# btracey/mpi

Measured on AMD Instinct MI355X. Metric: allreduce_sum_f32_256MiB algbw, higher is better.
Workload: dtype f32; 1 GPU; BASELINE cfg 4: allreduce-sum f32 256 MiB/rank, 8 ranks; ranks=8, ranks_per_gpu=8, bytes_per_rank=268435456, algo=auto (library), schedule_by=library defaults (ranks meet on the host: one schedule), transport=intra-HBM (all ranks share one GPU)

## Files before the change

mpi_amd/build.py:

```python
from __future__ import annotations

import hashlib
import json
import os
import shutil
import subprocess
import sys

ROOT = os.path.dirname(os.path.dirname(os.path.abspath(__file__)))
CSRC = os.path.join(ROOT, "mpi_amd", "csrc")
LIB = os.path.join(ROOT, "mpi_amd", "libxmpi.so")
HOSTLIB = os.path.join(ROOT, "mpi_amd", "libxmpi_host.so")
BIN = os.path.join(ROOT, "mpi_amd", "bin")

HIPCC = os.environ.get("HIPCC") or shutil.which("hipcc") or "/opt/rocm/bin/hipcc"
ARCH = "gfx950"
CXXFLAGS = ["-O3", "-std=c++17", "-fPIC", "-ffp-contract=off", "-Wall", "-Wextra"]

LIB_SOURCES = ["kernels.hip", "sched.hip", "ll.hip", "engine.cpp", "p2p.cpp", "agent.cpp", "api.cpp", "pool.cpp", "init.cpp", "tune.cpp", "local.cpp", "dump.cpp", "ctl.cpp", "ctl_selftest.cpp", "plan.cpp", "zcopy.cpp", "heap.cpp", "dsync.cpp", "dsync_conn.cpp", "trace.cpp"]
LIB_HEADERS = ["kernels.h", "kdev.h", "sched_steps.h", "comm.h", "ctl.h", "plan.h", "trace.h", os.path.join("..", "..", "include", "xmpi.h"),
               os.path.join("..", "..", "include", "xmpi_test.h")]


MANIFEST = os.path.join(ROOT, "mpi_amd", ".build_manifest.json")
# ... 80 lines not shown
    if os.path.exists(mpi_cpp):
        deps = [mpi_cpp, net_cpp, os.path.join(host_dir, "mpi.hpp"), os.path.join(host_dir, "network.hpp"),
                os.path.join(host_dir, "gobwire.hpp"), os.path.join(ROOT, "include", "xmpi.h"),
                os.path.join(ROOT, "include", "xmpi_test.h")]
        if force or _newer(HOSTLIB, deps):
            _run(["g++", "-O2", "-std=c++17", "-fPIC", "-ffp-contract=off", "-fno-fast-math", "-Wall", "-Wextra", "-shared", *inc, mpi_cpp, net_cpp, "-o", HOSTLIB,
                  "-L", os.path.dirname(LIB), "-lxmpi", "-Wl,-rpath,$ORIGIN", "-lpthread"], HOSTLIB, deps)
        outs.append(HOSTLIB)
        for name, src in (("helloworld", os.path.join(ROOT, "examples", "helloworld.cpp")),
                          ("bounce", os.path.join(ROOT, "examples", "bounce.cpp")),
                          ("allreduce", os.path.join(ROOT, "examples", "allreduce.cpp")),
                          ("coll_sweep", os.path.join(ROOT, "examples", "coll_sweep.cpp")),
                          ("allreduce_bench", os.path.join(ROOT, "examples", "allreduce_bench.cpp")),
                          ("cfg5_sweep", os.path.join(ROOT, "examples", "cfg5_sweep.cpp")),
                          ("cfg3_allgather", os.path.join(ROOT, "examples", "cfg3_allgather.cpp")),
                          ("alltoall", os.path.join(ROOT, "examples", "alltoall.cpp"))):
            if os.path.exists(src):
                out = os.path.join(BIN, name)
                if force or _newer(out, [src] + deps):
                    _run(["g++", "-O2", "-std=c++17", "-Wall", "-Wextra", *inc, src, "-o", out, "-L",
                          os.path.dirname(LIB), "-lxmpi_host", "-lxmpi", "-Wl,-rpath,$ORIGIN/..", "-lpthread"],
                         out, [src] + deps)
                outs.append(out)
    launcher = os.path.join(ROOT, "launcher", "xmpirun.cpp")
    if os.path.exists(launcher):
        out = os.path.join(BIN, "xmpirun")
        if force or _newer(out, [launcher]):
            _run(["g++", "-O2", "-std=c++17", "-Wall", "-Wextra", launcher, "-o", out], out, [launcher])
        outs.append(out)
    return outs


def build_oracle(force: bool = False) -> list[str]:
    odir = os.path.join(ROOT, "oracle")
    outs = []
    src = os.path.join(odir, "xmpi_oracle.c")
    out = os.path.join(odir, "liboracle.so")
    if force or _newer(out, [src, os.path.join(odir, "xmpi_oracle.h")]):
        _run(["gcc", "-O2", "-std=c11", "-fPIC", "-shared", "-ffp-contract=off", "-fno-fast-math", "-Wall",
              "-Wextra", src, "-o", out, "-lm"], out, [src, os.path.join(odir, "xmpi_oracle.h")])
    outs.append(out)
    ref = os.path.join(odir, "refpath.cpp")
    if os.path.exists(ref):
        out = os.path.join(odir, "librefpath.so")
        if force or _newer(out, [ref, os.path.join(odir, "gob_codec.h")]):
            _run(["g++", "-O2", "-std=c++17", "-fPIC", "-shared", "-Wall", "-Wextra", ref, "-o", out, "-lpthread"],
# ... 56 lines not shown
```

mpi_amd/csrc/api.cpp:

```cpp
#include <algorithm>
#include <cstdio>
#include <cstdlib>
#include <cstring>
#include <mutex>
#include <string>

#include "comm.h"
#include "kernels.h"

namespace xmpi {

static thread_local std::string g_last_error;
thread_local uint64_t t_api_call = 0;

void set_last_error(const std::string& s) { g_last_error = s; }

int hip_fail(hipError_t e, const char* what, const char* file, int line) {
  const char* base = strrchr(file, '/');
  g_last_error = std::string(what) + " failed: " + hipGetErrorString(e) + " (" + (base ? base + 1 : file) + ":" +
                 std::to_string(line) + ")";
  (void)hipGetLastError();
  return XMPI_ERR_HIP;
}

// ... 66 lines not shown
  }
  c->wq_cv.notify_all();
  return r;
}

void drain_worker(xmpi_comm* c) {
  if (t_in_worker || !c->worker_started) return;
  std::unique_lock<std::mutex> l(c->wq_mu);
  c->wq_cv.wait(l, [c] { return c->wq_busy == 0; });
}

void stop_worker(xmpi_comm* c) {
  if (!c->worker_started) return;
  drain_worker(c);
  {
    std::lock_guard<std::mutex> l(c->wq_mu);
    c->wq_stop = true;
  }
  c->wq_cv.notify_all();
  c->worker.join();
  c->worker_started = false;
}

static int collective_on_host_meeting_ranks(xmpi_comm* c, int coll, int algo, int root, const void* sendbuf, void* recvbuf, size_t count, int dtype,
                                            int op) {
  const size_t es = xmpi_dtype_size((xmpi_dtype)dtype);
  const bool zc_algo = algo == XMPI_ALGO_ZCOPY || algo == XMPI_ALGO_ZPUSH || algo == XMPI_ALGO_LL;
  if (c->size > 1 && (zc_algo || (algo == XMPI_ALGO_AUTO && c->zero_copy))) {
    bool done = false;
    int zrc = zero_copy_collective(c, coll, root, sendbuf, recvbuf, count, dtype, op, algo == XMPI_ALGO_ZPUSH, &done);
    if (zrc != XMPI_OK || done) return zrc;
  }
  if (zc_algo) algo = XMPI_ALGO_AUTO;
  if (algo == XMPI_ALGO_RING_PUSH) algo = XMPI_ALGO_RING;
  if (algo == XMPI_ALGO_RHD_PUSH) algo = XMPI_ALGO_RHD;
  if (algo == XMPI_ALGO_TREE_PUSH) algo = XMPI_ALGO_TREE;
  PlanParams pp;
  pp.coll = coll;
  pp.algo = algo;
  pp.size = c->size;
  pp.rank = c->rank;
  pp.root = root;
  pp.count = count;
  pp.elem_size = es;
  pp.channels = c->channels > 0 ? (int)c->channels : ring_channel_count(c->size);
  pp.lanes = c->lanes;
  const size_t total = count * es;
  size_t chunk = total;
  if (coll == COLL_ALLREDUCE) chunk = total / (size_t)c->size / (size_t)std::max(1, pp.channels);
  pp.piece_bytes = choose_piece(c, chunk);
  pp.fuse = 1;
  pp.fifo_depth = c->fifo_depth;
  pp.oneshot_bytes = (size_t)std::max<long>(0, c->oneshot_bytes);
  Plan plan;
  int rc = build_plan(pp, &plan);
// ... 65 lines not shown
  RoctxRange range("xmpi:%s algo=%s bytes=%zu rank=%d/%d", coll_name(coll), algo_name(algo), count * es, c->rank, c->size);
  std::lock_guard<std::mutex> g(c->coll_mu);
  if (dsync_takes(c, coll, algo))
    return dsync_collective(c, coll, root, sendbuf, recvbuf, count, dtype, op, c->local_stream, true, algo);
  const bool send_host = !is_device_pointer(sendbuf), recv_host = !is_device_pointer(recvbuf);
  if (send_host || recv_host) {
    const size_t send_bytes = coll_send_bytes(coll, c->size, count * es), recv_bytes = coll_recv_bytes(coll, c->size, count * es);
    const bool in_place = sendbuf == recvbuf && coll != COLL_ALLGATHER;
    void* up_recv = recv_host ? heap_alloc(c->device, recv_bytes) : nullptr;
    void* up_send = send_host && !(in_place && recv_host) ? heap_alloc(c->device, send_bytes) : nullptr;
    if ((recv_host && !up_recv) || (send_host && !(in_place && recv_host) && !up_send)) {
      if (up_recv) (void)heap_free(up_recv);
      if (up_send) (void)heap_free(up_send);
      (void)hipGetLastError();
      return collective_on_host_meeting_ranks(c, coll, algo, root, sendbuf, recvbuf, count, dtype, op);
    }
    void* drecv = recv_host ? up_recv : recvbuf;
    const void* dsend = !send_host ? sendbuf : (in_place && recv_host) ? drecv : up_send;
    auto done = [&](int rc) {
      if (up_recv) (void)heap_free(up_recv);
      if (up_send) (void)heap_free(up_send);
      return rc;
    };
    hipStream_t s = c->local_stream;
    const void* src_up = coll == COLL_BCAST ? (c->rank == root && recv_host ? recvbuf : nullptr) : (send_host ? sendbuf : nullptr);
    void* dst_up = coll == COLL_BCAST ? drecv : const_cast<void*>(dsend);
    if (src_up) {
      if (hipMemcpyAsync(dst_up, src_up, send_bytes, hipMemcpyHostToDevice, s) != hipSuccess || hipStreamSynchronize(s) != hipSuccess)
        return done(hip_fail(hipGetLastError(), "hipMemcpyAsync(host slice -> its stand-in)", __FILE__, __LINE__));
    }
    int rc = collective_on_host_meeting_ranks(c, coll, algo, root, dsend, drecv, count, dtype, op);
    if (rc == XMPI_OK && recv_host && (coll != COLL_REDUCE || c->rank == root)) {
      if (hipMemcpyAsync(recvbuf, drecv, recv_bytes, hipMemcpyDeviceToHost, s) != hipSuccess || hipStreamSynchronize(s) != hipSuccess)
        rc = hip_fail(hipGetLastError(), "hipMemcpyAsync(stand-in -> host slice)", __FILE__, __LINE__);
    }
    return done(rc);
  }
  return collective_on_host_meeting_ranks(c, coll, algo, root, sendbuf, recvbuf, count, dtype, op);
}

}

using namespace xmpi;

static int why_peer(xmpi_comm* c, int rc, const char* what) {
  if (rc == XMPI_ERR_PEER && c->ctl) set_last_error(std::string(what) + ": " + c->ctl->abort_reason());
  return rc;
}

extern "C" {

size_t xmpi_dtype_size(xmpi_dtype dtype) {
  switch (dtype) {
    case XMPI_U8: return 1;
    case XMPI_I32: return 4;
    case XMPI_I64: return 8;
    case XMPI_F16: return 2;
// ... 485 lines not shown
    const int rc = collective(c, COLL_ALLREDUCE, algo, 0, sendbuf, recvbuf, count, (int)dtype, (int)op);
    if (rc != XMPI_OK) return rc;
  }
  return XMPI_OK;
}

int xmpi_heap_selftest(uint64_t seed, int rounds) { return heap_selftest(seed, rounds); }


int xmpi_set_param(xmpi_comm* c, const char* name, long value) {
  if (!c || c->finalized || !name) return XMPI_ERR_STATE;
  std::lock_guard<std::mutex> g(c->coll_mu);
  const std::string n = name;
  if (n == "channels") c->channels = std::max<long>(0, value);
  else if (n == "piece_bytes") c->piece_bytes = std::max<long>(0, value);
  else if (n == "copy_engine") c->copy_engine = value ? 1 : 0;
  else if (n == "timeout_s") c->timeout_s = value;
  else if (n == "prof_every") c->prof_every = std::max<long>(1, value);
  else if (n == "batch_copies") c->batch_copies = value ? 1 : 0;
  else if (n == "oneshot_bytes") c->oneshot_bytes = std::max<long>(0, value);
  else if (n == "zero_copy") c->zero_copy = value ? 1 : 0;
  else if (n == "zc_bcast_push_bytes") c->zc_bcast_push_bytes = std::max<long>(0, value);
  else if (n == "zc_group_launch") c->zc_group_launch = value ? 1 : 0;
  else if (n == "p2p_direct_bytes") c->p2p_direct_bytes = value;
  else if (n == "p2p_kernel_ack") c->p2p_kernel_ack = value ? 1 : 0;
  else if (n == "p2p_agent_us") c->p2p_agent_us = std::max<long>(0, value);
  else if (n == "dsync") c->dsync = value ? 1 : 0;
  else if (n == "dsync_grid") c->dsync_grid_cap = std::max<long>(0, value);
  else if (n == "dsync_unroll") c->dsync_unroll = std::max<long>(1, std::min<long>(2, value));
  else if (n == "dsync_tiles") c->dsync_tiles = std::max<long>(1, value);
  else if (n == "p2p_grid_cap") c->p2p_grid_cap = std::max<long>(0, std::min<long>(value, 4096));
  else if (n == "ll_bytes") c->ll_bytes = std::max<long>(0, std::min<long>((long)kLLMaxPayload, value));
  else if (n == "agent_ll") c->agent_ll = value < 0 ? 0 : std::min<long>(value, 2);
  else if (n == "ll_agent_us") c->ll_agent_us = std::max<long>(0, value);
  else if (n == "agent_ll_bytes") c->agent_ll_bytes = std::max<long>(0, std::min<long>((long)kLLMaxPayload, value));
  else if (n == "dsync_split_bytes") c->dsync_split_bytes = std::max<long>(0, value);
  else if (n == "xcd_check") c->xcd_check = value ? 1 : 0;
  else if (n == "body_sys") c->body_sys = value ? 1 : 0;
  else if (n == "xcds") c->xcds = (int)std::max<long>(0, std::min<long>(value, 32));
  else if (n == "sched_channels") c->sched_channels = std::max<long>(0, value);
  else if (n == "sched_grid") c->sched_grid = std::max<long>(0, value);
  else if (n == "tree_piece_bytes") c->tree_piece_bytes = std::max<long>(4096, value);
  else if (n == "tuned") c->tuned = value != 0;
  else if (n == "tune_mask") c->tune_mask = value;
  else if (n.rfind("tune_", 0) == 0) {
    int coll = -1, cls = -1;
// ... 95 lines not shown
  if (n == "tune_check_us") return (long)(c->tune_check_ms * 1e3);
  if (n.rfind("tune_", 0) == 0) {
    int coll = -1, cls = -1;
    char what[16] = {0};
    if (sscanf(name, "tune_%15[a-z]_%d_%d", what, &coll, &cls) == 3 && coll >= 0 && coll < 4 && cls >= 0 && cls < xmpi_comm::kTuneClasses) {
      const std::string w = what;
      if (w == "algo") return c->tune_algo[coll][cls];
      if (w == "split") return c->tune_split[coll][cls];
      if (w == "unroll") return c->tune_unroll[coll][cls];
    }
    return -1;
  }
  if (n.rfind("prof_min_ns_", 0) == 0 || n.rfind("prof_max_ns_", 0) == 0) {
    const int kind = name[12] - '0';
    if (kind < 0 || kind >= PROF_KINDS || name[13]) return -1;
    return (long)((n[6] == 'i' ? c->prof[kind].min_ms : c->prof[kind].max_ms) * 1e6);
  }
  if (n == "p2p_direct_count") return (long)c->p2p_direct_count;
  if (n == "p2p_staged_count") return (long)c->p2p_staged_count;
  if (n == "p2p_lane_count") return (long)c->p2p_lane_count;
  if (n == "host_bounce_calls") return (long)c->host_bounce_calls;
  if (n == "host_lane_bytes") return (long)c->ctl->host_lane_bytes();
  if (n == "zc_seq") return (long)c->zc_seq;
  if (n == "zc_fallbacks_unregistered") return (long)c->zc_fallbacks_unregistered;
  if (n == "zc_fallbacks_unmappable") return (long)c->zc_fallbacks_unmappable;
  if (n == "shared_stream") return c->shared_stream ? 1 : 0;
  if (n == "kernel_mode") return get_kernel_mode();
  if (n == "last_run_us") return (long)c->last_run_us;
  if (n == "last_sync_us") return (long)c->last_sync_us;
  if (n == "lanes") return c->lanes;
  if (n == "fifo_depth") return c->fifo_depth;
  if (n == "slot_bytes") return (long)c->slot_bytes;
  if (n == "p2p_slot_bytes") return (long)c->p2p_slot_bytes;
  if (n == "window_bytes") return (long)c->window_bytes;
  if (n == "ring_channels_max") return ring_channel_count(c->size) * c->lanes;
  if (n == "ring_channels") return ring_channel_count(c->size);
  return -1;
}

}
```

mpi_amd/csrc/comm.h:

```cpp
#pragma once
#include <hip/hip_runtime_api.h>

#include <atomic>
#include <condition_variable>
#include <cstring>
#include <deque>
#include <functional>
#include <map>
#include <thread>
#include <mutex>
#include <set>
#include <string>
#include <utility>
#include <vector>

#include "../../include/xmpi.h"
#include "../../include/xmpi_test.h"
#include "ctl.h"
#include "kernels.h"
#include "trace.h"
#include "plan.h"

namespace xmpi {

// ... 45 lines not shown
  std::string degraded_why;

  int lanes = 2, fifo_depth = 8, p2p_depth = 2;
  size_t slot_bytes = 4u << 20, p2p_slot_bytes = 4u << 20;
  size_t coll_region_bytes = 0;
  size_t coll_slot_off(int src, int lane, uint64_t seq) const {
    return (((size_t)src * lanes + lane) * fifo_depth + (size_t)(seq % (uint64_t)fifo_depth)) * slot_bytes;
  }
  size_t p2p_slot_off(int src, int entry, uint64_t seq) const {
    return coll_region_bytes +
           (((size_t)src * xmpi::kMailEntries + entry) * p2p_depth + (size_t)(seq % (uint64_t)p2p_depth)) *
               p2p_slot_bytes;
  }

  hipStream_t send_stream[xmpi::kMaxRanks] = {nullptr};
  hipStream_t recv_stream[xmpi::kMaxRanks] = {nullptr};
  hipStream_t local_stream = nullptr;
  hipStream_t batch_send_stream = nullptr, batch_recv_stream = nullptr;
  long zero_copy = 1;
  long zc_bcast_push_bytes = 256 << 10;
  long zc_group_launch = 1;
  uint64_t zc_fallbacks_unregistered = 0, zc_fallbacks_unmappable = 0;
  uint64_t zc_seq = 0;
  std::set<std::pair<uint64_t, uint64_t>> zc_announced;
  std::mutex zc_mu;
  long p2p_direct_bytes = 1;
  uint64_t p2p_direct_count = 0, p2p_staged_count = 0, p2p_lane_count = 0;
  uint64_t zc_retired_seen[xmpi::kMaxRanks] = {0};
  long oneshot_bytes = 1 << 20;
  long batch_copies = 1;
  bool shared_stream = false;
  bool staged_streams = false;
  bool peer_coloc[xmpi::kMaxRanks] = {false};
  long prof_every = 1;
  uint64_t prof_seq[xmpi::PROF_KINDS] = {0};

  long dsync = 1;
  bool dsync_ok = false;
  xmpi::DsyncPage* dpage = nullptr;
  xmpi::DsyncPage* peer_page[xmpi::kMaxRanks] = {nullptr};
  bool peer_page_opened[xmpi::kMaxRanks] = {false};
  const int32_t* dsync_abort_dev = nullptr;
  char* ctl_dev = nullptr;
  bool ctl_registered = false;
  xmpi::DsyncResolved* dsync_res = nullptr;
  hipEvent_t dsync_order_ev = nullptr;
// ... 134 lines not shown

  std::mutex ev_mu;
  std::vector<hipEvent_t> ev_free, ev_timed_free;

  bool prof_on = false;
  xmpi::ProfCounter prof[xmpi::PROF_KINDS];

  std::mutex coll_mu;
  std::mutex p2p_mu;
  std::set<std::pair<int, int>> send_tags, recv_tags;
  std::map<std::pair<int, int>, xmpi::MailEntry*> pending_sends;
  std::vector<hipStream_t> p2p_streams;

  std::thread worker;
  std::mutex wq_mu;
  std::condition_variable wq_cv;
  std::deque<std::pair<std::function<int()>, xmpi_request*>> wq;
  size_t wq_busy = 0;
  bool wq_stop = false, worker_started = false;
  bool finalized = false;
};

namespace xmpi {
int ensure_streams(xmpi_comm* c);
int run_plan(xmpi_comm* c, const Plan& plan, const void* sendbuf, void* recvbuf, int dtype, int op);
int p2p_send(xmpi_comm* c, const void* buf, size_t bytes, int dtype, int dest, int tag, bool wait_ack = true);
int p2p_wait(xmpi_comm* c, int dest, int tag);
int p2p_recv(xmpi_comm* c, void* buf, size_t cap_bytes, int dtype, int src, int tag, size_t* got_bytes);
int p2p_probe(xmpi_comm* c, int src, int tag, size_t* bytes, int* dtype);
bool agent_submit(xmpi_comm* c, void* dst, const void* from, size_t bytes, MailEntry* m);
void p2p_agent_stop(xmpi_comm* c);
int agent_submit_ll(xmpi_comm* c, const void* send, void* recv, size_t bytes, int ll_coll, int root, int dtype, int op, bool consecutive);
extern thread_local uint64_t t_api_call;
void ll_agent_stop(xmpi_comm* c);
int zero_copy_collective(xmpi_comm* c, int coll, int root, const void* sendbuf, void* recvbuf, size_t count,
                         int dtype, int op, bool push, bool* done, int iters = 1);
int registry_add(void* base, size_t bytes, int device);
void registry_remove(xmpi_comm* c, void* base);
void zc_close_peers(const xmpi_comm* c);
bool zc_export(xmpi_comm* c, const void* p, size_t need, BufRef* ref);
bool zc_import(xmpi_comm* c, int peer, const BufRef& ref, void** out);
bool registry_alive(uint64_t gen);
hipError_t ipc_open_shared(int owner_pid, uint64_t owner_addr, const void* handle_bytes, void** out);
void ipc_close_shared(void* ptr);
void* pool_acquire(int device, size_t bytes, int kind, bool* fresh, uint64_t* mark);
void pool_release(void* ptr, uint64_t mark = 0);
hipError_t pool_handle(void* ptr, void* handle_out);
hipStream_t stream_acquire(int device);
void stream_release(int device, hipStream_t s);
hipStream_t shared_stream_for(int device);
bool trace_on();
#define XMPI_TRACE_STEP(rank, what)                                                                          \
  do {                                                                                                       \
    if (::xmpi::trace_on()) fprintf(stderr, "[xmpi %d %.6f] %s\n", (rank), ::xmpi::now_seconds(), (what)); \
  } while (0)
long env_long(const char* name, long dflt);
inline int use_device(const xmpi_comm* c) {
  XMPI_HIP(hipSetDevice(c->device));
  return XMPI_OK;
}
#define XMPI_ENTER(c)                          \
  do {                                         \
    if (!(c) || (c)->finalized) {              \
      ::xmpi::set_last_error("communicator not initialised"); \
      return XMPI_ERR_STATE;                   \
    }                                          \
    int _rc = ::xmpi::use_device(c);           \
    if (_rc) return _rc;                       \
    ::xmpi::t_api_call = (c)->api_calls.fetch_add(1, std::memory_order_relaxed) + 1; \
  } while (0)
inline double wait_limit(const xmpi_comm* c) { return c->timeout_s > 0 ? (double)c->timeout_s : 1e18; }
void drain_worker(xmpi_comm* c);
void stop_worker(xmpi_comm* c);
// ... 47 lines not shown
```

mpi_amd/csrc/ctl.h:

```cpp
#pragma once
#include <atomic>
#include <cstddef>
#include <cstdint>
#include <string>

namespace xmpi {

constexpr int kMaxRanks = 16;
constexpr int kMaxLanes = 4;
constexpr int kMailEntries = 4;
constexpr int kHostLaneSlots = 4;
constexpr uint64_t kCtlMagic = 0x584D504943544C31ull;
constexpr uint32_t kCtlVersion = 11;

struct alignas(64) Counter {
  std::atomic<uint64_t> v;
  char pad[56];
};

struct PipeCtl {
  Counter head;
  Counter tail;
};

enum MailState : uint32_t { MAIL_FREE = 0, MAIL_CLAIMED = 1, MAIL_POSTED = 2, MAIL_MATCHED = 3, MAIL_DONE = 4 };

struct BufRef {
  uint64_t base;
  uint64_t gen;
  uint64_t offset;
  uint64_t bytes;
  uint8_t handle[64];
};

enum MailDirect : int32_t {
  DIRECT_NONE = 0,
// ... 21 lines not shown
  int32_t device;
  int32_t maps;
  uint64_t window_addr;
  uint64_t window_bytes;
  uint8_t ipc_handle[64];
  char busid[32];
  uint64_t flag_addr;
  uint64_t flag_epoch;
  uint8_t flag_handle[64];
  char maps_why[96];
  int64_t ll_choice;
  uint64_t start_time;
};
constexpr int32_t kMapsWindows = 1, kMapsFlags = 2;

struct alignas(64) BufDesc {
  std::atomic<uint64_t> seq;
  int32_t ok;
  int32_t fresh;
  std::atomic<int32_t> verdict;
  int32_t in_place;
  BufRef send, recv;
  uint32_t sig;
};
static_assert(sizeof(BufDesc) == 256, "a descriptor is four cache lines");

constexpr int kRetireRing = 512;
struct alignas(64) RetireLog {
  std::atomic<uint64_t> count;
  uint64_t gen[kRetireRing];
};

constexpr int kPubRing = 64;
struct PubEntry {
  uint64_t gen;
  uint64_t base;
  uint64_t bytes;
  uint64_t reserved;
  uint8_t handle[64];
};
struct alignas(64) PubTable {
  std::atomic<uint64_t> count;
  char pad[56];
  PubEntry e[kPubRing];
};

// ... 101 lines not shown
```

mpi_amd/csrc/init.cpp:

```cpp
#include <unistd.h>

#include <algorithm>
#include <cstdlib>
#include <cstring>
#include <string>

#include "comm.h"
#include "kernels.h"

namespace xmpi {
namespace {

void* zeroed_device_words(size_t bytes, hipStream_t s) {
  void* p = nullptr;
  if (hipMalloc(&p, bytes) == hipSuccess) (void)hipMemsetAsync(p, 0, bytes, s);
  else p = nullptr;
  (void)hipGetLastError();
  return p;
}

void release_mappings_and_streams(xmpi_comm* c) {
  zc_close_peers(c);
  dsync_finalize(c);
  for (int p = 0; p < c->size; p++) {
// ... 42 lines not shown
    (void)hipGetLastError();
    set_last_error("xmpi_init: no HIP device is visible; xmpi has no CPU fallback");
    return XMPI_ERR_NOGPU;
  }
  if (*device < 0) *device = rank % ndev;
  if (*device >= ndev) {
    set_last_error("xmpi_init: device " + std::to_string(*device) + " does not exist (" + std::to_string(ndev) + " visible)");
    return XMPI_ERR_ARG;
  }
  XMPI_HIP(hipSetDevice(*device));
  return XMPI_OK;
}

void read_env(xmpi_comm* c) {
  c->timeout_s = std::max<long>(0, env_long("XMPI_TIMEOUT_S", 0));
  c->channels = env_long("XMPI_CHANNELS", 0);
  c->piece_bytes = env_long("XMPI_PIECE_BYTES", 0);
  c->copy_engine = env_long("XMPI_COPY_ENGINE", 0);
  c->batch_copies = env_long("XMPI_BATCH_COPIES", 1) ? 1 : 0;
  c->oneshot_bytes = std::max<long>(0, env_long("XMPI_ONESHOT_BYTES", 1 << 20));
  c->zero_copy = env_long("XMPI_ZERO_COPY", 1) ? 1 : 0;
  c->zc_bcast_push_bytes = std::max<long>(0, env_long("XMPI_ZC_BCAST_PUSH_BYTES", 256 << 10));
  c->zc_group_launch = env_long("XMPI_ZC_GROUP_LAUNCH", 1) ? 1 : 0;
  c->p2p_direct_bytes = env_long("XMPI_P2P_DIRECT_BYTES", 1);
  if (getenv("XMPI_KERNEL_MODE")) set_kernel_mode((int)env_long("XMPI_KERNEL_MODE", -1));
  if (getenv("XMPI_GRID_CAP")) set_grid_cap((int)env_long("XMPI_GRID_CAP", 0));
  c->dsync = env_long("XMPI_DSYNC", 1) ? 1 : 0;
  c->dsync_split_bytes = std::max<long>(0, env_long("XMPI_DSYNC_SPLIT_BYTES", 4 << 20));
  c->xcd_check = env_long("XMPI_XCD_CHECK", 1) ? 1 : 0;
  c->body_sys = env_long("XMPI_BODY_SYS", -1);
  c->ll_bytes = env_long("XMPI_LL_BYTES", -1);
  c->agent_ll = std::max<long>(0, std::min<long>(env_long("XMPI_AGENT_LL", 1), 2));
  c->agent_ll_bytes = std::max<long>(0, std::min<long>((long)kLLMaxPayload, env_long("XMPI_AGENT_LL_BYTES", 8192)));
  c->sched_channels = std::max<long>(0, env_long("XMPI_SCHED_CHANNELS", 0));
  c->sched_grid = std::max<long>(0, env_long("XMPI_SCHED_GRID", 0));
  c->tree_piece_bytes = std::max<long>(4096, env_long("XMPI_TREE_PIECE_BYTES", 256 << 10));
  c->dsync_grid_cap = std::max<long>(0, env_long("XMPI_DSYNC_GRID", 0));
  c->p2p_kernel_ack = env_long("XMPI_P2P_KERNEL_ACK", 1) ? 1 : 0;
  c->p2p_agent_us = std::max<long>(0, env_long("XMPI_P2P_AGENT_US", 40));
  c->ll_agent_us = std::max<long>(0, env_long("XMPI_LL_AGENT_US", c->p2p_agent_us));
  c->p2p_grid_cap = std::max<long>(0, std::min<long>(env_long("XMPI_P2P_GRID_CAP", 0), 4096));
  c->watchdog_ms = std::max<long>(0, env_long("XMPI_WATCHDOG_MS", 50));
  c->selfcheck = env_long("XMPI_SELFCHECK", -1);
}

int join_job(int rank, int size, int device, const char* job_key, double limit, xmpi_comm** out) {
// ... 276 lines not shown
```

mpi_amd/csrc/pool.cpp:

```cpp
#include <signal.h>

#include <cerrno>
#include <cstring>
#include <mutex>
#include <vector>

#include "comm.h"

namespace xmpi {

struct IpcMapping {
  int owner_pid;
  uint64_t owner_addr;
  uint8_t handle[64];
  void* ptr;
  int refs;
};
static std::mutex g_ipc_mu;
static std::vector<IpcMapping> g_ipc_map;

hipError_t ipc_open_shared(int owner_pid, uint64_t owner_addr, const void* handle_bytes, void** out) {
  std::lock_guard<std::mutex> g(g_ipc_mu);
  for (size_t i = 0; i < g_ipc_map.size(); i++) {
    IpcMapping& m = g_ipc_map[i];
// ... 155 lines not shown
int ensure_streams(xmpi_comm* c) {
  if (c->shared_stream || c->staged_streams) return XMPI_OK;
  bool ok = (c->batch_send_stream = stream_acquire(c->device)) && (c->batch_recv_stream = stream_acquire(c->device));
  for (int p = 0; p < c->size && ok; p++) {
    if (p == c->rank) continue;
    ok = (c->send_stream[p] = stream_acquire(c->device)) && (c->recv_stream[p] = stream_acquire(c->device));
  }
  if (!ok) return hip_fail(hipGetLastError(), "hipStreamCreate", __FILE__, __LINE__);
  c->staged_streams = true;
  return XMPI_OK;
}

hipStream_t shared_stream_for(int device) {
  static std::mutex mu;
  static std::vector<std::pair<int, hipStream_t>> streams;
  std::lock_guard<std::mutex> g(mu);
  for (auto& kv : streams)
    if (kv.first == device) return kv.second;
  hipStream_t s = nullptr;
  if (hipStreamCreateWithFlags(&s, hipStreamNonBlocking) != hipSuccess) return nullptr;
  streams.push_back({device, s});
  return s;
}
}
```

mpi_amd/csrc/zcopy.cpp:

```cpp
#include <dirent.h>
#include <signal.h>
#include <unistd.h>

#include <cerrno>

#include <algorithm>
#include <atomic>
#include <cstdio>
#include <cstring>
#include <map>
#include <mutex>
#include <vector>

#include "comm.h"
#include "kernels.h"

namespace xmpi {
namespace {

struct Alloc {
  uint64_t base;
  size_t bytes;
  int device;
  uint64_t gen;
  bool have_handle;
  hipIpcMemHandle_t handle;
};
std::mutex g_reg_mu;
std::map<uint64_t, Alloc> g_reg;
uint64_t g_next_gen = 1;

bool registry_lookup(const void* p, size_t need, int device, Alloc* out) {
  std::lock_guard<std::mutex> g(g_reg_mu);
  const uint64_t a = (uint64_t)(uintptr_t)p;
// ... 91 lines not shown
    XMPI_HIP(hipEventRecord(fin, c->local_stream));
    Backoff bo;
    for (;;) {
      const hipError_t e = hipEventQuery(fin);
      if (e == hipSuccess) break;
      if (e != hipErrorNotReady) return hip_fail(e, "hipEventQuery", __FILE__, __LINE__);
      (void)hipGetLastError();
      bo.pause();
    }
    ev_put(c, fin, false);
    if (start) {
      float ms = 0.f;
      XMPI_HIP(hipEventElapsedTime(&ms, start, stop));
      ProfCounter& pc = c->prof[PROF_ZCOPY];
      pc.add(ms, bytes);
      ev_put(c, start, true);
      ev_put(c, stop, true);
      start = stop = nullptr;
    }
    return XMPI_OK;
  }
};

}

int registry_add(void* base, size_t bytes, int device) {
  std::lock_guard<std::mutex> g(g_reg_mu);
  Alloc al;
  memset(&al, 0, sizeof al);
  al.base = (uint64_t)(uintptr_t)base;
  al.bytes = bytes;
  al.device = device;
  al.gen = g_next_gen++;
  al.have_handle = false;
  g_reg[al.base] = al;
  return XMPI_OK;
}

void registry_remove(xmpi_comm* c, void* base) {
  std::lock_guard<std::mutex> g(g_reg_mu);
  auto it = g_reg.find((uint64_t)(uintptr_t)base);
  if (it == g_reg.end()) return;
  if (it->second.have_handle && c && c->ctl) {
    RetireLog* log = c->ctl->retired(c->rank);
    const uint64_t n = log->count.load(std::memory_order_relaxed);
    log->gen[n % kRetireRing] = it->second.gen;
// ... 61 lines not shown
  }
  drop_retired(c);
  void* base = nullptr;
  if (map_peer(pid, ref, &base) != hipSuccess) return false;
  *out = (char*)base + ref.offset;
  return true;
}

void zc_close_peers(const xmpi_comm* c) {
  (void)c;
  std::lock_guard<std::mutex> g(g_map_mu);
  for (size_t i = 0; i < g_maps.size();) {
    if (kill(g_maps[i].pid, 0) != 0 && errno == ESRCH) {
      (void)hipIpcCloseMemHandle(g_maps[i].ptr);
      g_maps.erase(g_maps.begin() + (long)i);
    } else {
      i++;
    }
  }
  (void)hipGetLastError();
}

static int zc_run(xmpi_comm* c, int coll, int root, const void* sendbuf, void* recvbuf, size_t count, int dtype,
                  int op, bool push, bool* done, int iters) {
  *done = false;
  const int N = c->size, me = c->rank;
  const size_t es = xmpi_dtype_size((xmpi_dtype)dtype);
  const size_t unit = count * es;
  const size_t send_bytes = coll_send_bytes(coll, N, unit), recv_bytes = coll_recv_bytes(coll, N, unit);
  const bool recv_significant = (coll != COLL_REDUCE) || me == root;

  const uint64_t seq = ++c->zc_seq;
  BufDesc* mine = c->ctl->desc(me, seq);
  bool fresh = false;
  bool ok = fill_ref(c, sendbuf, send_bytes, &mine->send, &fresh);
  if (recv_significant) ok = fill_ref(c, recvbuf, recv_bytes, &mine->recv, &fresh) && ok;
  else mine->recv = mine->send;
  mine->ok = ok ? 1 : 0;
  mine->fresh = fresh ? 1 : 0;
  mine->in_place = (sendbuf == recvbuf) ? 1 : 0;
  {
    const bool reduces = coll_reduces(coll), rooted = coll == COLL_BCAST || coll == COLL_REDUCE;
    uint64_t h = 0x9E3779B97F4A7C15ull;
    for (uint64_t v : {(uint64_t)coll + 1, (uint64_t)(push ? 2 : 1), (uint64_t)send_bytes, reduces ? (uint64_t)dtype + 1 : 0,
                       reduces ? (uint64_t)op + 1 : 0, rooted ? (uint64_t)root + 1 : 0, (uint64_t)iters}) {
      h = (h ^ v) * 0x100000001B3ull;
      h ^= h >> 29;
    }
    mine->sig = (uint32_t)(h ^ (h >> 32));
  }
  mine->verdict.store(0, std::memory_order_relaxed);
  mine->seq.store(seq, std::memory_order_release);
  int rc = c->ctl->barrier(wait_limit(c));
  if (rc != XMPI_OK) {
    set_last_error("zero-copy collective: a peer did not arrive");
    return rc;
  }

  drop_retired(c);

  bool all_ok = true, any_fresh = false, any_in_place = false;
  for (int p = 0; p < N; p++) {
    BufDesc* d = c->ctl->desc(p, seq);
    if (d->seq.load(std::memory_order_acquire) != seq) {
      set_last_error("zero-copy collective: ranks disagree on the collective sequence (mismatched calls?)");
      c->ctl->set_abort(XMPI_ERR_STATE);
      return XMPI_ERR_STATE;
    }
    if (d->sig != mine->sig) {
      set_last_error("collective: the ranks are not in the same call (collective, length, dtype, operation or root differ between "
                     "this rank and a peer); nothing was moved");
      c->ctl->set_abort(XMPI_ERR_ARG);
      return XMPI_ERR_ARG;
    }
    all_ok = all_ok && d->ok == 1;
    any_fresh = any_fresh || d->fresh == 1;
    any_in_place = any_in_place || d->in_place == 1;
  }
  if (!all_ok) {
    c->zc_fallbacks_unregistered++;
    return XMPI_OK;
  }

  const int mypid = (int)getpid();
  char* psend[kMaxRanks];
  char* precv[kMaxRanks];
  bool mapped = true;
  for (int p = 0; p < N && mapped; p++) {
    if (p == me) {
      psend[p] = (char*)const_cast<void*>(sendbuf);
      precv[p] = (char*)recvbuf;
      continue;
    }
    const BufDesc* d = c->ctl->desc(p, seq);
    const int pid = c->ctl->info(p)->pid;
    if (pid == mypid) {
      psend[p] = (char*)(uintptr_t)(d->send.base + d->send.offset);
      precv[p] = (char*)(uintptr_t)(d->recv.base + d->recv.offset);
      continue;
    }
// ... 10 lines not shown
        fprintf(stderr, "xmpi: rank %d cannot map a buffer of rank %d (pid %d): %s; %zu mappings open, %d fds open\n",
                me, p, pid, hipGetErrorString(me_err), g_maps.size(), count_open_fds());
    }
    if (mapped) {
      psend[p] = (char*)bs + d->send.offset;
      precv[p] = (char*)br + d->recv.offset;
    }
  }
  if (any_fresh) {
    mine->verdict.store(mapped ? 1 : -1, std::memory_order_release);
    rc = c->ctl->barrier(wait_limit(c));
    if (rc != XMPI_OK) return rc;
    for (int p = 0; p < N; p++)
      if (c->ctl->desc(p, seq)->verdict.load(std::memory_order_acquire) != 1) {
        c->zc_fallbacks_unmappable++;
        return XMPI_OK;
      }
  } else if (!mapped) {
    set_last_error("zero-copy collective: a peer buffer that was mapped before can no longer be mapped");
    c->ctl->set_abort(XMPI_ERR_HIP);
    return XMPI_ERR_HIP;
  }

  hipStream_t s = c->local_stream;
  Launcher L(c);
  const size_t al = std::max<size_t>(1, 16 / es);
  const bool use_push = push && coll == COLL_ALLREDUCE && !any_in_place && N > 1 && count % ((size_t)N * al) == 0;
  if (use_push) {
    const size_t C = count / (size_t)N, cb = C * es;
    {
      void* dst[kMaxBatch];
      const void* src[kMaxBatch];
      size_t bytes[kMaxBatch];
      int n = 0;
      for (int d = 1; d < N; d++) {
        const int q = (me + d) % N;
        dst[n] = precv[q] + (size_t)me * cb;
        src[n] = psend[me] + (size_t)q * cb;
        bytes[n] = cb;
        if (++n == kMaxBatch || d == N - 1) {
          rc = L.begin(2 * (size_t)n * cb);
          if (rc) return rc;
          XMPI_HIP(launch_copy_batch(dst, nullptr, src, bytes, n, s, L.start, L.stop));
          rc = L.finish();
          if (rc) return rc;
          n = 0;
// ... 5 lines not shown
    {
      const void* srcs[kMaxRanks];
      for (int p = 0; p < N; p++) srcs[p] = (p == me) ? psend[me] + (size_t)me * cb : precv[me] + (size_t)p * cb;
      void* d1[1] = {precv[me] + (size_t)me * cb};
      rc = L.begin((size_t)(N + 1) * cb);
      if (rc) return rc;
      XMPI_HIP(launch_reduce_n_multi(d1, 1, srcs, N, C, dtype, op, s, L.start, L.stop));
      rc = L.finish();
      if (rc) return rc;
    }
    rc = c->ctl->barrier(wait_limit(c));
    if (rc != XMPI_OK) return rc;
    {
      void* dsts[kMaxRanks];
      int nd = 0;
      for (int d = 1; d < N; d++) dsts[nd++] = precv[(me + d) % N] + (size_t)me * cb;
      rc = L.begin((size_t)(1 + nd) * cb);
      if (rc) return rc;
      XMPI_HIP(launch_copy_multi(dsts, nd, precv[me] + (size_t)me * cb, cb, s, L.start, L.stop));
      rc = L.finish();
      if (rc) return rc;
    }
  } else if (coll == COLL_ALLREDUCE || coll == COLL_REDUCE) {
    int lo = me, hi = me;
    if (c->zc_group_launch) {
      while (lo > 0 && c->peer_coloc[lo - 1]) lo--;
      while (hi + 1 < N && c->peer_coloc[hi + 1]) hi++;
    }
    size_t off = 0, cnt = 0, off_hi = 0, cnt_hi = 0;
    zc_chunk(count, es, N, lo, &off, &cnt);
    zc_chunk(count, es, N, hi, &off_hi, &cnt_hi);
    cnt = off_hi + cnt_hi - off;
    if (me == lo && cnt > 0) {
      const void* srcs[kMaxRanks];
      void* dsts[kMaxRanks];
      for (int p = 0; p < N; p++) srcs[p] = psend[p] + off * es;
      int nd = 0;
      if (coll == COLL_REDUCE) {
        dsts[nd++] = precv[root] + off * es;
      } else {
        dsts[nd++] = precv[me] + off * es;
        for (int d = 1; d < N; d++) dsts[nd++] = precv[(me + d) % N] + off * es;
      }
      std::vector<std::pair<hipEvent_t, hipEvent_t>> sampled;
      for (int it = 0; it < iters; it++) {
        rc = L.begin((size_t)(N + nd) * cnt * es);
        if (rc) return rc;
        XMPI_HIP(launch_reduce_n_multi(dsts, nd, srcs, N, cnt, dtype, op, s, L.start, L.stop));
        if (it + 1 < iters && L.start) {
          sampled.push_back({L.start, L.stop});
          L.start = L.stop = nullptr;
        }
      }
      rc = L.finish();
      if (rc) return rc;
      for (auto& ev : sampled) {
        float ms = 0.f;
        XMPI_HIP(hipEventElapsedTime(&ms, ev.first, ev.second));
        ProfCounter& pc = c->prof[PROF_ZCOPY];
        pc.add(ms, (size_t)(N + nd) * cnt * es);
        ev_put(c, ev.first, true);
        ev_put(c, ev.second, true);
      }
    }
  } else if (coll == COLL_REDUCE_SCATTER) {
    const void* srcs[kMaxRanks];
    for (int p = 0; p < N; p++) srcs[p] = psend[p] + (size_t)me * unit;
    void* d1[1] = {precv[me]};
    rc = L.begin((size_t)(N + 1) * unit);
    if (rc) return rc;
    XMPI_HIP(launch_reduce_n_multi(d1, 1, srcs, N, count, dtype, op, s, L.start, L.stop));
    rc = L.finish();
    if (rc) return rc;
  } else if (coll == COLL_ALLTOALL) {
    static_assert(kMaxRanks <= kMaxBatch, "one batch holds a pair per rank");
    void* dst[kMaxBatch];
    const void* src[kMaxBatch];
    size_t bytes[kMaxBatch];
    for (int d = 0; d < N; d++) {
      const int q = (me + d) % N;
      dst[d] = precv[q] + (size_t)me * unit;
      src[d] = psend[me] + (size_t)q * unit;
      bytes[d] = unit;
    }
    rc = L.begin(2 * (size_t)N * unit);
    if (rc) return rc;
    XMPI_HIP(launch_copy_batch(dst, nullptr, src, bytes, N, s, L.start, L.stop));
// ... 62 lines not shown
          if (q != root) dsts[nd++] = precv[q] + off * es;
        }
        if (cnt > 0 && nd > 0) {
          rc = L.begin((size_t)(1 + nd) * cnt * es);
          if (rc) return rc;
          XMPI_HIP(launch_copy_multi(dsts, nd, precv[me] + off * es, cnt * es, s, L.start, L.stop));
          rc = L.finish();
          if (rc) return rc;
        }
      }
    }
  }

  rc = c->ctl->barrier(wait_limit(c));
  if (rc != XMPI_OK) {
    set_last_error("zero-copy collective: a peer did not finish");
    return rc;
  }
  *done = true;
  return XMPI_OK;
}

int zero_copy_collective(xmpi_comm* c, int coll, int root, const void* sendbuf, void* recvbuf, size_t count,
                         int dtype, int op, bool push, bool* done, int iters) {
  RoctxRange range("xmpi:zcopy(host rendezvous) %s count=%zu x%d", coll_name(coll), count, iters);
  const int rc = zc_run(c, coll, root, sendbuf, recvbuf, count, dtype, op, push, done, iters);
  if (rc != XMPI_OK) c->ctl->set_abort(rc);
  return rc;
}

}
```

Before: 396.3 GB/s.

## Pipeline host-slice allreduce in pieces overlapping upload, reduce, and download

When allreduce buffers live in host memory, the zero-copy path now splits the work into fixed-size pieces (8 MiB by default). The host-to-device upload of the next piece is interleaved with the reduction of the current one, and a background thread copies finished pieces back to the host on a separate stream. This targets the serial upload, reduce and download sequence for host buffers. It adds two barriers per piece, a helper thread, and a descriptor field so all ranks agree on the piece size.

```diff
diff --git a/mpi_amd/build.py b/mpi_amd/build.py
--- a/mpi_amd/build.py
+++ b/mpi_amd/build.py
@@ -126,6 +126,12 @@
                           os.path.dirname(LIB), "-lxmpi_host", "-lxmpi", "-Wl,-rpath,$ORIGIN/..", "-lpthread"],
                          out, [src] + deps)
                 outs.append(out)
+    duplex = os.path.join(ROOT, "examples", "pcie_duplex.cpp")
+    if os.path.exists(duplex):
+        out = os.path.join(BIN, "pcie_duplex")
+        if force or _newer(out, [duplex]):
+            _run([HIPCC, f"--offload-arch={ARCH}", "-O2", "-std=c++17", "-Wall", "-Wextra", duplex, "-o", out, "-lpthread"], out, [duplex])
+        outs.append(out)
     launcher = os.path.join(ROOT, "launcher", "xmpirun.cpp")
     if os.path.exists(launcher):
         out = os.path.join(BIN, "xmpirun")
diff --git a/mpi_amd/csrc/api.cpp b/mpi_amd/csrc/api.cpp
--- a/mpi_amd/csrc/api.cpp
+++ b/mpi_amd/csrc/api.cpp
@@ -112,15 +112,40 @@
   c->worker_started = false;
 }
 
+int host_leg_up(xmpi_comm* c, HostLeg* leg, size_t upto) {
+  upto = std::min(upto, leg->bytes);
+  if (!leg->up_src || leg->up_done >= upto) return XMPI_OK;
+  hipStream_t up = nullptr, down = nullptr;
+  if (!host_leg_streams(c->device, &up, &down)) return hip_fail(hipGetLastError(), "hipStreamCreate(host leg)", __FILE__, __LINE__);
+  XMPI_HIP(hipMemcpyAsync(leg->up_dst + leg->up_done, leg->up_src + leg->up_done, upto - leg->up_done, hipMemcpyHostToDevice, up));
+  XMPI_HIP(hipStreamSynchronize(up));
+  leg->up_done = upto;
+  return XMPI_OK;
+}
+
+static int rc_up_rest(xmpi_comm* c, HostLeg* leg) {
+  const int rc = host_leg_up(c, leg, leg->bytes);
+  if (rc != XMPI_OK) c->ctl->set_abort(rc);
+  return rc;
+}
+
+static size_t host_piece_for(const xmpi_comm* c, int coll, int algo, size_t count, size_t es) {
+  if (coll != COLL_ALLREDUCE || c->host_piece_bytes <= 0 || c->size < 2 || t_in_worker) return 0;
+  if (!(algo == XMPI_ALGO_ZCOPY || algo == XMPI_ALGO_LL || (algo == XMPI_ALGO_AUTO && c->zero_copy))) return 0;
+  const size_t piece = std::max<size_t>(4096, (size_t)c->host_piece_bytes / 4096 * 4096);
+  return count * es > piece ? piece : 0;
+}
+
 static int collective_on_host_meeting_ranks(xmpi_comm* c, int coll, int algo, int root, const void* sendbuf, void* recvbuf, size_t count, int dtype,
-                                            int op) {
+                                            int op, HostLeg* leg = nullptr) {
   const size_t es = xmpi_dtype_size((xmpi_dtype)dtype);
   const bool zc_algo = algo == XMPI_ALGO_ZCOPY || algo == XMPI_ALGO_ZPUSH || algo == XMPI_ALGO_LL;
   if (c->size > 1 && (zc_algo || (algo == XMPI_ALGO_AUTO && c->zero_copy))) {
     bool done = false;
-    int zrc = zero_copy_collective(c, coll, root, sendbuf, recvbuf, count, dtype, op, algo == XMPI_ALGO_ZPUSH, &done);
+    int zrc = zero_copy_collective(c, coll, root, sendbuf, recvbuf, count, dtype, op, algo == XMPI_ALGO_ZPUSH, &done, 1, leg);
     if (zrc != XMPI_OK || done) return zrc;
   }
+  if (leg && (rc_up_rest(c, leg)) != XMPI_OK) return XMPI_ERR_HIP;
   if (zc_algo) algo = XMPI_ALGO_AUTO;
   if (algo == XMPI_ALGO_RING_PUSH) algo = XMPI_ALGO_RING;
   if (algo == XMPI_ALGO_RHD_PUSH) algo = XMPI_ALGO_RHD;
@@ -232,17 +257,34 @@
       if (up_send) (void)heap_free(up_send);
       return rc;
     };
+    auto failed = [&](const char* what) {
+      const int rc = hip_fail(hipGetLastError(), what, __FILE__, __LINE__);
+      c->ctl->set_abort(rc);
+      return done(rc);
+    };
     hipStream_t s = c->local_stream;
     const void* src_up = coll == COLL_BCAST ? (c->rank == root && recv_host ? recvbuf : nullptr) : (send_host ? sendbuf : nullptr);
     void* dst_up = coll == COLL_BCAST ? drecv : const_cast<void*>(dsend);
-    if (src_up) {
+    HostLeg leg;
+    leg.piece = host_piece_for(c, coll, algo, count, es);
+    if (leg.piece) {
+      leg.bytes = count * es;
+      leg.up_src = (const char*)src_up;
+      leg.up_dst = (char*)dst_up;
+      leg.down_dst = recv_host ? (char*)recvbuf : nullptr;
+      leg.down_src = (const char*)drecv;
+      if (host_leg_up(c, &leg, leg.piece) != XMPI_OK) {
+        c->ctl->set_abort(XMPI_ERR_HIP);
+        return done(XMPI_ERR_HIP);
+      }
+    } else if (src_up) {
       if (hipMemcpyAsync(dst_up, src_up, send_bytes, hipMemcpyHostToDevice, s) != hipSuccess || hipStreamSynchronize(s) != hipSuccess)
-        return done(hip_fail(hipGetLastError(), "hipMemcpyAsync(host slice -> its stand-in)", __FILE__, __LINE__));
-    }
-    int rc = collective_on_host_meeting_ranks(c, coll, algo, root, dsend, drecv, count, dtype, op);
-    if (rc == XMPI_OK && recv_host && (coll != COLL_REDUCE || c->rank == root)) {
+        return failed("hipMemcpyAsync(host slice -> its stand-in)");
+    }
+    int rc = collective_on_host_meeting_ranks(c, coll, algo, root, dsend, drecv, count, dtype, op, leg.piece ? &leg : nullptr);
+    if (rc == XMPI_OK && recv_host && !leg.down_done && (coll != COLL_REDUCE || c->rank == root)) {
       if (hipMemcpyAsync(recvbuf, drecv, recv_bytes, hipMemcpyDeviceToHost, s) != hipSuccess || hipStreamSynchronize(s) != hipSuccess)
-        rc = hip_fail(hipGetLastError(), "hipMemcpyAsync(stand-in -> host slice)", __FILE__, __LINE__);
+        return failed("hipMemcpyAsync(stand-in -> host slice)");
     }
     return done(rc);
   }
@@ -774,6 +816,7 @@
   else if (n == "zero_copy") c->zero_copy = value ? 1 : 0;
   else if (n == "zc_bcast_push_bytes") c->zc_bcast_push_bytes = std::max<long>(0, value);
   else if (n == "zc_group_launch") c->zc_group_launch = value ? 1 : 0;
+  else if (n == "host_piece_bytes") c->host_piece_bytes = std::max<long>(0, value);
   else if (n == "p2p_direct_bytes") c->p2p_direct_bytes = value;
   else if (n == "p2p_kernel_ack") c->p2p_kernel_ack = value ? 1 : 0;
   else if (n == "p2p_agent_us") c->p2p_agent_us = std::max<long>(0, value);
@@ -915,6 +958,8 @@
   if (n == "host_bounce_calls") return (long)c->host_bounce_calls;
   if (n == "host_lane_bytes") return (long)c->ctl->host_lane_bytes();
   if (n == "zc_seq") return (long)c->zc_seq;
+  if (n == "host_piece_bytes") return c->host_piece_bytes;
+  if (n == "host_pieces") return (long)c->host_pieces;
   if (n == "zc_fallbacks_unregistered") return (long)c->zc_fallbacks_unregistered;
   if (n == "zc_fallbacks_unmappable") return (long)c->zc_fallbacks_unmappable;
   if (n == "shared_stream") return c->shared_stream ? 1 : 0;
diff --git a/mpi_amd/csrc/comm.h b/mpi_amd/csrc/comm.h
--- a/mpi_amd/csrc/comm.h
+++ b/mpi_amd/csrc/comm.h
@@ -91,6 +91,8 @@
   long zc_group_launch = 1;
   uint64_t zc_fallbacks_unregistered = 0, zc_fallbacks_unmappable = 0;
   uint64_t zc_seq = 0;
+  long host_piece_bytes = 8 << 20;
+  uint64_t host_pieces = 0;
   std::set<std::pair<uint64_t, uint64_t>> zc_announced;
   std::mutex zc_mu;
   long p2p_direct_bytes = 1;
@@ -271,6 +273,17 @@
 };
 
 namespace xmpi {
+struct HostLeg {
+  const char* up_src = nullptr;
+  char* up_dst = nullptr;
+  char* down_dst = nullptr;
+  const char* down_src = nullptr;
+  size_t bytes = 0;
+  size_t piece = 0;
+  size_t up_done = 0;
+  bool down_done = false;
+};
+int host_leg_up(xmpi_comm* c, HostLeg* leg, size_t upto);
 int ensure_streams(xmpi_comm* c);
 int run_plan(xmpi_comm* c, const Plan& plan, const void* sendbuf, void* recvbuf, int dtype, int op);
 int p2p_send(xmpi_comm* c, const void* buf, size_t bytes, int dtype, int dest, int tag, bool wait_ack = true);
@@ -283,7 +296,7 @@
 extern thread_local uint64_t t_api_call;
 void ll_agent_stop(xmpi_comm* c);
 int zero_copy_collective(xmpi_comm* c, int coll, int root, const void* sendbuf, void* recvbuf, size_t count,
-                         int dtype, int op, bool push, bool* done, int iters = 1);
+                         int dtype, int op, bool push, bool* done, int iters = 1, HostLeg* leg = nullptr);
 int registry_add(void* base, size_t bytes, int device);
 void registry_remove(xmpi_comm* c, void* base);
 void zc_close_peers(const xmpi_comm* c);
@@ -298,6 +311,7 @@
 hipStream_t stream_acquire(int device);
 void stream_release(int device, hipStream_t s);
 hipStream_t shared_stream_for(int device);
+bool host_leg_streams(int device, hipStream_t* up, hipStream_t* down);
 bool trace_on();
 #define XMPI_TRACE_STEP(rank, what)                                                                          \
   do {                                                                                                       \
diff --git a/mpi_amd/csrc/ctl.h b/mpi_amd/csrc/ctl.h
--- a/mpi_amd/csrc/ctl.h
+++ b/mpi_amd/csrc/ctl.h
@@ -11,7 +11,7 @@
 constexpr int kMailEntries = 4;
 constexpr int kHostLaneSlots = 4;
 constexpr uint64_t kCtlMagic = 0x584D504943544C31ull;
-constexpr uint32_t kCtlVersion = 11;
+constexpr uint32_t kCtlVersion = 12;
 
 struct alignas(64) Counter {
   std::atomic<uint64_t> v;
@@ -79,6 +79,7 @@
   int32_t in_place;
   BufRef send, recv;
   uint32_t sig;
+  uint64_t host_piece;
 };
 static_assert(sizeof(BufDesc) == 256, "a descriptor is four cache lines");
 
diff --git a/mpi_amd/csrc/init.cpp b/mpi_amd/csrc/init.cpp
--- a/mpi_amd/csrc/init.cpp
+++ b/mpi_amd/csrc/init.cpp
@@ -88,6 +88,7 @@
   c->zero_copy = env_long("XMPI_ZERO_COPY", 1) ? 1 : 0;
   c->zc_bcast_push_bytes = std::max<long>(0, env_long("XMPI_ZC_BCAST_PUSH_BYTES", 256 << 10));
   c->zc_group_launch = env_long("XMPI_ZC_GROUP_LAUNCH", 1) ? 1 : 0;
+  c->host_piece_bytes = std::max<long>(0, env_long("XMPI_HOST_PIECE_BYTES", 8l << 20));
   c->p2p_direct_bytes = env_long("XMPI_P2P_DIRECT_BYTES", 1);
   if (getenv("XMPI_KERNEL_MODE")) set_kernel_mode((int)env_long("XMPI_KERNEL_MODE", -1));
   if (getenv("XMPI_GRID_CAP")) set_grid_cap((int)env_long("XMPI_GRID_CAP", 0));
diff --git a/mpi_amd/csrc/pool.cpp b/mpi_amd/csrc/pool.cpp
--- a/mpi_amd/csrc/pool.cpp
+++ b/mpi_amd/csrc/pool.cpp
@@ -201,4 +201,30 @@
   streams.push_back({device, s});
   return s;
 }
-}
+
+bool host_leg_streams(int device, hipStream_t* up, hipStream_t* down) {
+  struct Pair {
+    int device;
+    hipStream_t up, down;
+  };
+  static std::mutex mu;
+  static std::vector<Pair> pairs;
+  std::lock_guard<std::mutex> g(mu);
+  for (auto& p : pairs)
+    if (p.device == device) {
+      *up = p.up;
+      *down = p.down;
+      return true;
+    }
+  Pair p{device, nullptr, nullptr};
+  if (hipStreamCreateWithFlags(&p.up, hipStreamNonBlocking) != hipSuccess) return false;
+  if (hipStreamCreateWithFlags(&p.down, hipStreamNonBlocking) != hipSuccess) {
+    (void)hipStreamDestroy(p.up);
+    return false;
+  }
+  pairs.push_back(p);
+  *up = p.up;
+  *down = p.down;
+  return true;
+}
+}
diff --git a/mpi_amd/csrc/zcopy.cpp b/mpi_amd/csrc/zcopy.cpp
--- a/mpi_amd/csrc/zcopy.cpp
+++ b/mpi_amd/csrc/zcopy.cpp
@@ -6,10 +6,12 @@
 
 #include <algorithm>
 #include <atomic>
+#include <condition_variable>
 #include <cstdio>
 #include <cstring>
 #include <map>
 #include <mutex>
+#include <thread>
 #include <vector>
 
 #include "comm.h"
@@ -147,6 +149,132 @@
   }
 };
 
+
+int zc_fold(xmpi_comm* c, Launcher& L, int coll, int root, char* const* psend, char* const* precv, size_t first, size_t n, size_t es,
+            int dtype, int op, int iters) {
+  const int N = c->size, me = c->rank;
+  hipStream_t s = c->local_stream;
+  int rc = XMPI_OK;
+  int lo = me, hi = me;
+  if (c->zc_group_launch) {
+    while (lo > 0 && c->peer_coloc[lo - 1]) lo--;
+    while (hi + 1 < N && c->peer_coloc[hi + 1]) hi++;
+  }
+  size_t off = 0, cnt = 0, off_hi = 0, cnt_hi = 0;
+  zc_chunk(n, es, N, lo, &off, &cnt);
+  zc_chunk(n, es, N, hi, &off_hi, &cnt_hi);
+  cnt = off_hi + cnt_hi - off;
+  off += first;
+  if (me == lo && cnt > 0) {
+    const void* srcs[kMaxRanks];
+    void* dsts[kMaxRanks];
+    for (int p = 0; p < N; p++) srcs[p] = psend[p] + off * es;
+    int nd = 0;
+    if (coll == COLL_REDUCE) {
+      dsts[nd++] = precv[root] + off * es;
+    } else {
+      dsts[nd++] = precv[me] + off * es;
+      for (int d = 1; d < N; d++) dsts[nd++] = precv[(me + d) % N] + off * es;
+    }
+    std::vector<std::pair<hipEvent_t, hipEvent_t>> sampled;
+    for (int it = 0; it < iters; it++) {
+      rc = L.begin((size_t)(N + nd) * cnt * es);
+      if (rc) return rc;
+      XMPI_HIP(launch_reduce_n_multi(dsts, nd, srcs, N, cnt, dtype, op, s, L.start, L.stop));
+      if (it + 1 < iters && L.start) {
+        sampled.push_back({L.start, L.stop});
+        L.start = L.stop = nullptr;
+      }
+    }
+    rc = L.finish();
+    if (rc) return rc;
+    for (auto& ev : sampled) {
+      float ms = 0.f;
+      XMPI_HIP(hipEventElapsedTime(&ms, ev.first, ev.second));
+      ProfCounter& pc = c->prof[PROF_ZCOPY];
+      pc.add(ms, (size_t)(N + nd) * cnt * es);
+      ev_put(c, ev.first, true);
+      ev_put(c, ev.second, true);
+    }
+  }
+  return XMPI_OK;
+}
+
+struct Downloader {
+  xmpi_comm* c;
+  HostLeg* leg;
+  hipStream_t stream;
+  size_t piece;
+  std::mutex mu;
+  std::condition_variable cv;
+  size_t released = 0;
+  bool stop = false;
+  int rc = XMPI_OK;
+  hipError_t err = hipSuccess;
+  std::thread th;
+  void main() {
+    if (hipSetDevice(c->device) != hipSuccess) return fail(hipGetLastError());
+    for (size_t p = 0; p * piece < leg->bytes; p++) {
+      {
+        std::unique_lock<std::mutex> l(mu);
+        cv.wait(l, [&] { return stop || released > p; });
+        if (released <= p) return;
+      }
+      const size_t off = p * piece, len = std::min(piece, leg->bytes - off);
+      if (hipMemcpyAsync(leg->down_dst + off, leg->down_src + off, len, hipMemcpyDeviceToHost, stream) != hipSuccess ||
+          hipStreamSynchronize(stream) != hipSuccess)
+        return fail(hipGetLastError());
+    }
+  }
+  void fail(hipError_t e) {
+    err = e;
+    rc = XMPI_ERR_HIP;
+    c->ctl->set_abort(rc);
+  }
+  void release(size_t n) {
+    {
+      std::lock_guard<std::mutex> l(mu);
+      released = n;
+    }
+    cv.notify_one();
+  }
+  int join(int call_rc) {
+    if (!th.joinable()) return call_rc;
+    if (call_rc != XMPI_OK) {
+      std::lock_guard<std::mutex> l(mu);
+      stop = true;
+    }
+    cv.notify_one();
+    th.join();
+    if (rc != XMPI_OK && call_rc == XMPI_OK) return hip_fail(err, "hipMemcpyAsync(piece of a stand-in -> host slice)", __FILE__, __LINE__);
+    return call_rc;
+  }
+};
+
+int zc_pieced_allreduce(xmpi_comm* c, char* const* psend, char* const* precv, size_t count, size_t es, int dtype, int op, size_t piece,
+                        HostLeg* leg) {
+  const size_t total = count * es, npieces = (total + piece - 1) / piece, per = piece / es;
+  Launcher L(c);
+  Downloader dl{c, leg, nullptr, piece};
+  if (leg && leg->down_dst) {
+    hipStream_t up = nullptr;
+    if (!host_leg_streams(c->device, &up, &dl.stream)) return hip_fail(hipGetLastError(), "hipStreamCreate(host leg)", __FILE__, __LINE__);
+    dl.th = std::thread([&dl] { dl.main(); });
+  }
+  int rc = XMPI_OK;
+  for (size_t p = 0; p < npieces && rc == XMPI_OK; p++) {
+    rc = c->ctl->barrier(wait_limit(c));
+    if (rc == XMPI_OK) rc = zc_fold(c, L, COLL_ALLREDUCE, 0, psend, precv, p * per, std::min(per, count - p * per), es, dtype, op, 1);
+    if (rc == XMPI_OK) rc = c->ctl->barrier(wait_limit(c));
+    if (rc != XMPI_OK) break;
+    dl.release(p + 1);
+    c->host_pieces++;
+    if (leg) rc = host_leg_up(c, leg, (p + 2) * piece);
+  }
+  rc = dl.join(rc);
+  if (rc == XMPI_OK && leg) leg->down_done = true;
+  return rc;
+}
 }
 
 int registry_add(void* base, size_t bytes, int device) {
@@ -254,7 +382,7 @@
 }
 
 static int zc_run(xmpi_comm* c, int coll, int root, const void* sendbuf, void* recvbuf, size_t count, int dtype,
-                  int op, bool push, bool* done, int iters) {
+                  int op, bool push, bool* done, int iters, HostLeg* leg) {
   *done = false;
   const int N = c->size, me = c->rank;
   const size_t es = xmpi_dtype_size((xmpi_dtype)dtype);
@@ -271,6 +399,7 @@
   mine->ok = ok ? 1 : 0;
   mine->fresh = fresh ? 1 : 0;
   mine->in_place = (sendbuf == recvbuf) ? 1 : 0;
+  mine->host_piece = leg ? leg->piece : 0;
   {
     const bool reduces = coll_reduces(coll), rooted = coll == COLL_BCAST || coll == COLL_REDUCE;
     uint64_t h = 0x9E3779B97F4A7C15ull;
@@ -292,6 +421,7 @@
   drop_retired(c);
 
   bool all_ok = true, any_fresh = false, any_in_place = false;
+  size_t piece = 0;
   for (int p = 0; p < N; p++) {
     BufDesc* d = c->ctl->desc(p, seq);
     if (d->seq.load(std::memory_order_acquire) != seq) {
@@ -308,6 +438,13 @@
     all_ok = all_ok && d->ok == 1;
     any_fresh = any_fresh || d->fresh == 1;
     any_in_place = any_in_place || d->in_place == 1;
+    if (d->host_piece && piece && d->host_piece != piece) {
+      set_last_error("allreduce on host slices: the ranks ask for different piece sizes (host_piece_bytes / XMPI_HOST_PIECE_BYTES differ "
+                     "between ranks); nothing was moved");
+      c->ctl->set_abort(XMPI_ERR_ARG);
+      return XMPI_ERR_ARG;
+    }
+    if (d->host_piece) piece = (size_t)d->host_piece;
   }
   if (!all_ok) {
     c->zc_fallbacks_unregistered++;
@@ -364,6 +501,11 @@
     return XMPI_ERR_HIP;
   }
 
+  if (piece) {
+    rc = zc_pieced_allreduce(c, psend, precv, count, es, dtype, op, piece, leg);
+    *done = rc == XMPI_OK;
+    return rc;
+  }
   hipStream_t s = c->local_stream;
   Launcher L(c);
   const size_t al = std::max<size_t>(1, 16 / es);
@@ -415,47 +557,8 @@
       if (rc) return rc;
     }
   } else if (coll == COLL_ALLREDUCE || coll == COLL_REDUCE) {
-    int lo = me, hi = me;
-    if (c->zc_group_launch) {
-      while (lo > 0 && c->peer_coloc[lo - 1]) lo--;
-      while (hi + 1 < N && c->peer_coloc[hi + 1]) hi++;
-    }
-    size_t off = 0, cnt = 0, off_hi = 0, cnt_hi = 0;
-    zc_chunk(count, es, N, lo, &off, &cnt);
-    zc_chunk(count, es, N, hi, &off_hi, &cnt_hi);
-    cnt = off_hi + cnt_hi - off;
-    if (me == lo && cnt > 0) {
-      const void* srcs[kMaxRanks];
-      void* dsts[kMaxRanks];
-      for (int p = 0; p < N; p++) srcs[p] = psend[p] + off * es;
-      int nd = 0;
-      if (coll == COLL_REDUCE) {
-        dsts[nd++] = precv[root] + off * es;
-      } else {
-        dsts[nd++] = precv[me] + off * es;
-        for (int d = 1; d < N; d++) dsts[nd++] = precv[(me + d) % N] + off * es;
-      }
-      std::vector<std::pair<hipEvent_t, hipEvent_t>> sampled;
-      for (int it = 0; it < iters; it++) {
-        rc = L.begin((size_t)(N + nd) * cnt * es);
-        if (rc) return rc;
-        XMPI_HIP(launch_reduce_n_multi(dsts, nd, srcs, N, cnt, dtype, op, s, L.start, L.stop));
-        if (it + 1 < iters && L.start) {
-          sampled.push_back({L.start, L.stop});
-          L.start = L.stop = nullptr;
-        }
-      }
-      rc = L.finish();
-      if (rc) return rc;
-      for (auto& ev : sampled) {
-        float ms = 0.f;
-        XMPI_HIP(hipEventElapsedTime(&ms, ev.first, ev.second));
-        ProfCounter& pc = c->prof[PROF_ZCOPY];
-        pc.add(ms, (size_t)(N + nd) * cnt * es);
-        ev_put(c, ev.first, true);
-        ev_put(c, ev.second, true);
-      }
-    }
+    rc = zc_fold(c, L, coll, root, psend, precv, 0, count, es, dtype, op, iters);
+    if (rc) return rc;
   } else if (coll == COLL_REDUCE_SCATTER) {
     const void* srcs[kMaxRanks];
     for (int p = 0; p < N; p++) srcs[p] = psend[p] + (size_t)me * unit;
@@ -564,9 +667,9 @@
 }
 
 int zero_copy_collective(xmpi_comm* c, int coll, int root, const void* sendbuf, void* recvbuf, size_t count,
-                         int dtype, int op, bool push, bool* done, int iters) {
+                         int dtype, int op, bool push, bool* done, int iters, HostLeg* leg) {
   RoctxRange range("xmpi:zcopy(host rendezvous) %s count=%zu x%d", coll_name(coll), count, iters);
-  const int rc = zc_run(c, coll, root, sendbuf, recvbuf, count, dtype, op, push, done, iters);
+  const int rc = zc_run(c, coll, root, sendbuf, recvbuf, count, dtype, op, push, done, iters, leg);
   if (rc != XMPI_OK) c->ctl->set_abort(rc);
   return rc;
 }
```

Result: slower. 390.6 GB/s (-1.4%).
